# prototypefund/your-voice-TTS

Measured on AMD Instinct MI355X. Metric: mel-frames/sec + RTF, Tacotron2 + 60-iter Griffin-Lim, LJSpeech, higher is better.
Workload: dtype f32; 1 GPU; configs[1]: Tacotron2 single sentence, HIP decoder loop + HIP Griffin-Lim 60 iters; sentences_per_gpu=1, L=100, gl_iters=60, model_config=config_tacotron2.json + forward_attn_mask (synthesize.py:86), parallelism=single GPU

## Files before the change

### your-voice-tts_amd/csrc/resident_decoder.hip

```cpp
#include "handoff.h"
#include "resident.h"

namespace tts {
namespace {
using namespace handoff;

__device__ __forceinline__ float lstm_cell16(float pre, float& c) {
    const int k = threadIdx.x;
    const float act = (k >> 2) == 2 ? tanh_cell(pre) : sigmoid_cell(pre);
    const float f = dpp_move<0x104, 0xf>(act, 0.f);
    const float g = dpp_move<0x108, 0xf>(act, 0.f);
    const float o = dpp_move<0x10C, 0xf>(act, 0.f);
    const float c2 = f * c + act * g;
    c = c2;
    return o * tanh_cell(c2);
}
__device__ __forceinline__ float sigmoid_fast(float x) {
    return __builtin_amdgcn_rcpf(1.f + __builtin_amdgcn_exp2f(-x * 1.4426950408889634f));
}

__device__ __forceinline__ float dot4(float4 w, float4 x, float acc) {
    acc = fmaf(w.x, x.x, acc);
    acc = fmaf(w.y, x.y, acc);
    acc = fmaf(w.z, x.z, acc);
    return fmaf(w.w, x.w, acc);
}
__device__ __forceinline__ float4 ld4(const float* p) { return *reinterpret_cast<const float4*>(p); }
__device__ __forceinline__ float sum32_dpp(float v) {
    v += dpp_move<0x111, 0xf>(v, 0.f);
    v += dpp_move<0x112, 0xf>(v, 0.f);
    v += dpp_move<0x114, 0xf>(v, 0.f);
    v += dpp_move<0x118, 0xf>(v, 0.f);
    v += dpp_move<0x142, 0xa>(v, 0.f);
    return v;
}

__device__ __forceinline__ int res_window(int k, int nn, int L) {
    if (k == 0) return nn >= 2 ? nn - 2 : nn - 2 + L;
    const int clo = nn >= 1 ? nn - 1 : L - 1, chi = min(nn + 2, L - 1);
    const int p = clo + k - 1;
    return p <= chi ? p : -1;
}
__device__ __forceinline__ int res_candidate(int s, int nn, int np, int L) {
    if (s < 5) return res_window(s, nn, L);
    if (s >= 15) return -1;
    const int p = res_window((s - 5) >> 1, np, L);
    if (p < 0) return -1;
    const int q = p + ((s - 5) & 1);
    return q < L ? q : -1;
}

constexpr int SM_WDL = 16 * 16 * 32 * 4;
constexpr int SM_ST = 64;
constexpr int SM_RQ = 4 * 64 * 4;
constexpr int SM_RM = 2 * 6 * 64 * 4 + 2 * 256;
constexpr int SM_PROF = 2 * 16;
constexpr int SM_FLOATS = SM_WDL + HATT + HDEC + (ENC + 16) + PRE + ADIM + 16 + 16 + SM_ST + SM_RQ + SM_RM + SM_PROF + PRE;
static_assert(SM_RM >= 6 * 64 * 4 + RES_WAVES * RES_LMAX, "attention CU partials");
static_assert(SM_RQ >= 3 * RES_LMAX + 2 * RES_WAVES + 16 + ADIM, "attention CU scratch");
static_assert(SM_RQ >= 2 * (RES_LMAX + 32) + RES_LMAX + RES_WAVES, "general attention form: weights, energies");
static_assert(SM_RM >= 2 * 6 * 64 * 4 + RES_LMAX + 32, "general attention form: cumulative weights");
static_assert(RES_LMAX == 4 * 64 && RES_LMAX == 32 * RES_WAVES, "4 positions per lane, one per wave of 32 CUs");

template <bool PROF, bool GEN>
__global__ __launch_bounds__(RES_THREADS, 1) void resident_decoder_kernel(const ResArgs a) {
    const int c = blockIdx.x;
    const int tid = threadIdx.x, lane = tid & 63;
    const int wave = __builtin_amdgcn_readfirstlane(tid >> 6);
    const int r = tid >> 5, ks = tid & 31;
    extern __shared__ __align__(16) float sm[];
    float4* wdl = reinterpret_cast<float4*>(sm);
    float* xh_att = sm + SM_WDL;
    float* xh_dec = xh_att + HATT;
    float* xctx = xh_dec + HDEC;
    float* xpre = xctx + ENC + 16;
    float* xq = xpre + PRE;
    float* gates = xq + ADIM;
    int* flags = reinterpret_cast<int*>(gates + 16);
    float* st = gates + 32;
    float* rq = st + SM_ST;
    float* rm = rq + SM_RQ;
    float* abuf = rq;
    float* an = abuf + 2 * RES_LMAX;
    float* scr = an + RES_LMAX;
    float* xv = scr + 2 * RES_WAVES + 16;
    float* red = rm + 6 * 64 * 4;
    long long* pacc = reinterpret_cast<long long*>(rm + SM_RM);
    float* xp1 = rm + SM_RM + SM_PROF;
    constexpr int GW_PAD = RES_LMAX + 32;
    float* gw = rq;
    float* geg = rq + 2 * GW_PAD;
    float* gts = geg + RES_LMAX;
    float* gcum = rm + 2 * 6 * 64 * 4;
    bool prof = false;
    long long plast = 0;
    long long* trace = PROF && a.prof ? a.prof + 2 * RES_PHASES + (size_t)c * RES_TRACE_STEPS * RES_TRACE_EV : nullptr;
#define RES_EV(t, k)                                                                                \
    if (PROF && trace && (t) < RES_TRACE_STEPS) trace[(t) * RES_TRACE_EV + (k)] = (long long)wall_clock64();
#define RES_MARK(k)                                     \
    if (PROF && prof && tid == 0) {                     \
        const long long now = (long long)wall_clock64(); \
        pacc[k] += now - plast;                         \
        plast = now;                                    \
    }

    float4 wa[14], wdc[4];
    constexpr int KF = HDEC + ENC;
    {
        const float4* p = a.w.wa + (size_t)c * 14 * RES_THREADS + tid;
#pragma unroll
        for (int i = 0; i < 14; ++i) wa[i] = p[(size_t)i * RES_THREADS];
        const float4* q = a.w.wdc + (size_t)c * 4 * RES_THREADS + tid;
#pragma unroll
        for (int i = 0; i < 4; ++i) wdc[i] = q[(size_t)i * RES_THREADS];
        if (wave == 2 && c < a.nmel)
            for (int i = 0; i < 6; ++i) reinterpret_cast<float4*>(rm)[i * 64 + lane] = ld4(a.w.wf + (size_t)c * KF + i * 256 + lane * 4);
        const float4* l = a.w.wdl + (size_t)c * (SM_WDL / 4);
        for (int i = tid; i < SM_WDL / 4; i += RES_THREADS) wdl[i] = l[i];
    }
    if (tid < 16) {
        st[tid] = a.w.ba[c * 16 + tid];
        st[16 + tid] = a.w.bd[c * 16 + tid];
    }
    if (tid < 4) {
        st[32 + tid] = a.c_att[4 * c + tid];
        st[36 + tid] = a.c_dec[4 * c + tid];
    }
    if (tid == 0) st[48] = c < a.nmel ? a.w.bf[c] : 0.f;
    if (tid == 1) st[49] = a.w.bf[a.nmel + PRE];
    for (int k = tid; k < HATT; k += RES_THREADS) {
        xh_att[k] = a.h_att[a.hps + k];
        xh_dec[k] = a.h_dec[a.hps + k];
    }
    for (int k = tid; k < ENC; k += RES_THREADS) xctx[k] = a.xa[PRE + k];
    if (tid == 0) {
        flags[0] = 0;
        flags[1] = 0;
        for (int k = 0; k < RES_PHASES; ++k) pacc[k] = 0;
    }
    __syncthreads();
    const long long tmo = a.timeout_ticks;
    int xcc;
    asm volatile("s_getreg_b32 %0, hwreg(HW_REG_XCC_ID)" : "=s"(xcc));
    xcc &= 7;
    const unsigned setup_tag = (a.salt << 14) | 0x3FFFu;
    if (tid == 0) publish(a.gran + GR_SETUP + c, setup_tag, __int_as_float(xcc));
    if (wave == 0) {
        float v4[4];
        const bool ok = sweep<4>(a.gran, setup_tag, v4, [&](int i) { return GR_SETUP + lane * 4 + i; }, tmo);
        int rank = 0, nx = 0, nmin = RES_CUS, nmax = 0;
        const int xref = __builtin_amdgcn_readfirstlane(__float_as_int(v4[0]) & 7);
        for (int k = 0; k < 8; ++k) {
            int cnt = 0;
#pragma unroll
            for (int i = 0; i < 4; ++i) {
                const int x = __float_as_int(v4[i]) & 7;
                cnt += __popcll(__ballot(x == k));
                if (k == xcc) rank += __popcll(__ballot(x == k && lane * 4 + i < c));
            }
            if (k == xcc) nx = cnt;
            if (cnt > 0) nmin = min(nmin, cnt);
            nmax = max(nmax, cnt);
        }
        if (GEN && nmax > RES_MIN_CUS_PER_XCD) nmin = 0;
        if (lane == 0) {
            int* fl = reinterpret_cast<int*>(flags);
            fl[2] = rank;
            fl[3] = nx;
            fl[4] = xref;
            if (!ok) { flags[1] = 1; fail(a.status, 6); }
            else if (nmin < RES_MIN_CUS_PER_XCD) { flags[1] = 1; fail(a.status, RES_STATUS_PLACEMENT); }
        }
    }
    __syncthreads();
    if (flags[1]) return;
    const int rank = flags[2], nx = flags[3];
    const int p2lo = rank * PRE / nx, p2hi = (rank + 1) * PRE / nx;
    const int r0 = p2lo + wave;
    const bool has_row = r0 < p2hi;
    const float4 wp0 = has_row ? ld4(a.w.w2 + r0 * PRE + lane * 4) : float4{0.f, 0.f, 0.f, 0.f};
    const float bp1 = has_row ? a.w.bf[a.nmel + r0] : 0.f;
    const float bp2 = has_row ? a.w.b2[r0] : 0.f;
    const float* w1p = a.w.wf + (size_t)(a.nmel + (has_row ? r0 : 0)) * KF + lane * 4;
    const bool stop_cu = rank == 0;
    if (stop_cu && wave == 3)
        for (int i = 0; i < 6; ++i)
            reinterpret_cast<float4*>(rm)[(6 + i) * 64 + lane] = ld4(a.w.wf + (size_t)(a.nmel + PRE) * KF + i * 256 + lane * 4);
    const int qrow = 4 * rank + (wave >> 1), qhalf = wave & 1;
    const float4 wq0 = ld4(a.w.wq + qrow * HATT + qhalf * 512 + lane * 4);
    const float4 wq1 = ld4(a.w.wq + qrow * HATT + qhalf * 512 + 256 + lane * 4);
    const int L = a.L;
    const bool att_cu = !GEN && rank == nx - 1;
    const bool xlog = xcc == flags[4];
    const bool att_log = att_cu && xlog;
    prof = PROF && a.prof != nullptr && a.prof_marks && (c == 0 || att_log);
    if (prof && tid == 0) plast = (long long)wall_clock64();
    int n = 0, n_prev = 0;
    float ufa = 0.f, vb = 0.f, ex = 0.f, erow[4] = {0.f, 0.f, 0.f, 0.f}, ptc[4] = {0.f, 0.f, 0.f, 0.f};
    const auto renc = __builtin_amdgcn_make_buffer_rsrc(const_cast<float*>(a.enc), (short)0, L * ENC * 4, 0x00020000);
    const auto rpt = __builtin_amdgcn_make_buffer_rsrc(const_cast<float*>(a.Pt), (short)0, ADIM * a.Lcap * 4, 0x00020000);
    auto prefetch_rows = [&](int nn) {
        const int cx = (nn - 2 + L) % L, clo = nn >= 1 ? nn - 1 : L - 1, chi = min(nn + 2, L - 1);
        ex = __uint_as_float(__builtin_amdgcn_raw_buffer_load_b32(renc, (cx * ENC + tid) * 4, 0, VOLATILE_AUX));
#pragma unroll
        for (int k = 0; k < 4; ++k)
            erow[k] = __uint_as_float(__builtin_amdgcn_raw_buffer_load_b32(
                renc, clo + k <= chi ? ((clo + k) * ENC + tid) * 4 : OOB_OFF, 0, VOLATILE_AUX));
    };
    if (att_cu) {
        n = a.nidx[0];
        ufa = a.u[0];
        vb = a.v_b[0];
        for (int j = tid; j < L; j += RES_THREADS) abuf[j] = a.alpha[j];
        if (tid < ADIM) xv[tid] = a.v[tid];
        prefetch_rows(n);
    }
    const int gf = GEN ? a.gen : 0;
    const int s_e = GR_EX + xcc * RES_LMAX;
    float gu = 0.5f, gtb = 0.f;
    int gwin = -1, gn = 1;
    float gv0 = 0.f, gv1 = 0.f, gp0 = 0.f, gp1 = 0.f, gl0 = 0.f, gl1 = 0.f;
    float gtw[3];
#pragma unroll
    for (int k = 0; k < 3; ++k) gtw[k] = 0.f;
    auto gen_location = [&](const float* wrow) {
        const int pe = rank + 32 * wave;
        if (pe >= L) return;
        const float* src = (lane < 32 ? wrow : gcum) + pe + 1;
        const float4* wc = reinterpret_cast<const float4*>(a.loc_conv) + lane * 8;
        float sacc = 0.f;
#pragma unroll
        for (int q = 0; q < 8; q += 2) {
            const float4 w0 = wc[q], w1_ = wc[q + 1];
            sacc = fmaf(w0.x, src[4 * q], sacc);
            sacc = fmaf(w0.y, src[4 * q + 1], sacc);
            sacc = fmaf(w0.z, src[4 * q + 2], sacc);
            sacc = fmaf(w0.w, src[4 * q + 3], sacc);
            sacc = fmaf(w1_.x, src[4 * q + 4], sacc);
            sacc = fmaf(w1_.y, src[4 * q + 5], sacc);
            sacc = fmaf(w1_.z, src[4 * q + 6], sacc);
            sacc = fmaf(w1_.w, src[4 * q + 7], sacc);
            asm volatile("" ::: "memory");
        }
        const float tot = sacc + __shfl_xor(sacc, 32, 64);
        const float4* wd0 = reinterpret_cast<const float4*>(a.loc_dense + lane * NLOC);
        const float4* wd1 = reinterpret_cast<const float4*>(a.loc_dense + (lane + 64) * NLOC);
        float l0 = 0.f, l1 = 0.f;
#pragma unroll
        for (int q = 0; q < 8; ++q) {
            const float4 u0 = wd0[q], u1 = wd1[q];
            const float f0 = __int_as_float(__builtin_amdgcn_readlane(__float_as_int(tot), 4 * q));
            const float f1 = __int_as_float(__builtin_amdgcn_readlane(__float_as_int(tot), 4 * q + 1));
            const float f2 = __int_as_float(__builtin_amdgcn_readlane(__float_as_int(tot), 4 * q + 2));
            const float f3 = __int_as_float(__builtin_amdgcn_readlane(__float_as_int(tot), 4 * q + 3));
            l0 = fmaf(u0.x, f0, l0); l0 = fmaf(u0.y, f1, l0); l0 = fmaf(u0.z, f2, l0); l0 = fmaf(u0.w, f3, l0);
            l1 = fmaf(u1.x, f0, l1); l1 = fmaf(u1.y, f1, l1); l1 = fmaf(u1.z, f2, l1); l1 = fmaf(u1.w, f3, l1);
            asm volatile("" ::: "memory");
        }
        gl0 = l0;
        gl1 = l1;
    };
    if constexpr (GEN) {
        vb = a.v_b[0];
        gu = a.u[0];
        gn = a.nidx[0];
        if (gf & GEN_WINDOW) gwin = a.win0[0];
        if (gf & GEN_TA) {
            gtb = a.ta_b[0];
#pragma unroll
            for (int k = 0; k < 3; ++k) gtw[k] = a.ta_w[3 * tid + k];
        }
        gv0 = a.v[lane];
        gv1 = a.v[lane + 64];
        const int pe = rank + 32 * wave;
        if (pe < L) {
            gp0 = a.Pt[(int64_t)lane * a.Lcap + pe];
            gp1 = a.Pt[(int64_t)(lane + 64) * a.Lcap + pe];
        }
        for (int k = tid; k < GW_PAD; k += RES_THREADS) {
            const int j = k - 16;
            const bool ok = j >= 0 && j < L;
            gw[k] = ok ? a.alpha[j] : 0.f;
            gw[GW_PAD + k] = ok && (gf & GEN_LOCATION) ? a.att_w0[j] : 0.f;
            gcum[k] = ok && (gf & GEN_LOCATION) ? a.att_cum0[j] : 0.f;
        }
        __syncthreads();
        if (gf & GEN_LOCATION) gen_location(gw + GW_PAD);
    }
    const bool stop_lane = stop_cu && wave == 3 && lane == 0;
    if (stop_lane) {
// ... 22 lines not shown
    int t = 0;
    for (;; ++t) {
        u64* G = a.gran + (t & 1) * GR_TOTAL;
        const unsigned E = (a.salt << 14) | (((unsigned)t & 2047u) << 3);
        const unsigned EP6 = ((a.salt << 14) | (((unsigned)(t - 1) & 2047u) << 3)) + 6u;
        float aa[2] = {0.f, 0.f};
#pragma unroll
        for (int i = 2; i < 6; ++i) aa[i & 1] = dot4(wa[i], ld4(xctx + (i - 2) * 128 + ks * 4), aa[i & 1]);
#pragma unroll
        for (int i = 6; i < 10; ++i) aa[i & 1] = dot4(wa[i], ld4(xh_att + (i - 6) * 128 + ks * 4), aa[i & 1]);
        asm volatile("" ::: "memory");
#pragma unroll
        for (int i = 10; i < 14; ++i) aa[i & 1] = dot4(wa[i], ld4(xh_att + (i - 6) * 128 + ks * 4), aa[i & 1]);
        float acc_a = aa[0] + aa[1];
        float ad[2] = {0.f, 0.f};
#pragma unroll 2
        for (int i = 8; i < 16; ++i)
            ad[i & 1] = dot4(wdl[(i * 16 + r) * 32 + ks], ld4(xh_dec + (i - 8) * 128 + ks * 4), ad[i & 1]);
        float acc_d = ad[0] + ad[1];
        if (wave < 3) {
            const int gp = s_1 + ((t & 1) ^ 1) * GR_TOTAL;
            bool ok = true;
            if (t == 0) {
                if (wave == 0) {
                    const float4 v = ld4(a.pre1 + lane * 4);
                    xp1[lane * 4] = v.x; xp1[lane * 4 + 1] = v.y; xp1[lane * 4 + 2] = v.z; xp1[lane * 4 + 3] = v.w;
                }
            } else {
                float p0 = 0.f, p1 = 0.f;
                for (int i = 0; i < a.sleep_p1; ++i) __builtin_amdgcn_s_sleep(4);
                if (wave < 2) {
                    ok = sweep_pair(rg, gp + 2 * pk, true, EP6, p0, p1, tmo);
                    xp1[2 * pk] = p0;
                    xp1[2 * pk + 1] = p1;
                } else {
                    ok = sweep_pair(rg, lane == 0 ? gp + PRE : -1, false, EP6, p0, p1, tmo);
                    if (lane == 0 && ok && p0 == 0.f) flags[0] = 1;
                }
            }
            RES_MARK(0);
            if (lane == 0 && !ok) { flags[1] = 1; fail(a.status, 1, t); }
        }
        __syncthreads();
        if (tid == 0) { RES_EV(t, 0) }
        if (flags[0] | flags[1]) break;
        {
            const float4 x = ld4(xp1 + lane * 4);
            u64* gx = Gx + (t & 1) * GR_TOTAL;
            if (has_row) {
                const float s0 = wave_sum_dpp(dot4(wp0, x, 0.f));
                if (lane == 0) publish_xcd(gx + r0, E + 1, fmaxf(s0 + bp2, 0.f));
            }
            RES_MARK(1);
            if (wave < 2) {
                for (int i = 0; i < a.sleep_pre2; ++i) __builtin_amdgcn_s_sleep(4);
                float q0, q1;
                const bool ok = sweep_pair(rg, s_x + (t & 1) * GR_TOTAL + 2 * pk, true, E + 1, q0, q1, tmo);
                xpre[2 * pk] = q0;
                xpre[2 * pk + 1] = q1;
                if (!ok && lane == 0) { flags[1] = 1; fail(a.status, 7, t); }
            }
        }
        __syncthreads();
        if (tid == 0) { RES_EV(t, 1) }
        if (flags[1]) break;
        RES_MARK(2);
#pragma unroll
        for (int i = 0; i < 2; ++i) acc_a = dot4(wa[i], ld4(xpre + i * 128 + ks * 4), acc_a);
        acc_a = sum32_dpp(acc_a);
        if (ks == 31) gates[r] = acc_a;
        __syncthreads();
        RES_MARK(3);
        if (tid < 16) {
            float cs = st[32 + (tid & 3)];
            const float h = lstm_cell16(gates[tid] + st[tid], cs);
            if (tid < 4) {
                st[32 + tid] = cs;
                st[40 + tid] = h;
                publish(G + GR_HATT + 4 * c + tid, E + 2, h);
                if (tid == 0) { RES_EV(t, 2) }
            }
        }
        if (att_cu && t > 0) {
            prefetch_rows(n);
            const int pos = res_candidate(tid >> 5, n, n_prev, L);
#pragma unroll
            for (int m = 0; m < 4; ++m)
                ptc[m] = __uint_as_float(__builtin_amdgcn_raw_buffer_load_b32(
                    rpt, pos >= 0 ? (((tid & 31) + 32 * m) * a.Lcap + pos) * 4 : OOB_OFF, 0, VOLATILE_AUX));
        }
        {
            if (wave == 4 && t > 0) mel_row(t - 1);
            for (int i = 0; i < a.sleep_hatt; ++i) __builtin_amdgcn_s_sleep(4);
            float h0, h1;
            const bool ok = sweep_pair(rg, (t & 1) * GR_TOTAL + GR_HATT + 2 * pk, true, E + 2, h0, h1, tmo);
            xh_att[2 * pk] = h0;
            xh_att[2 * pk + 1] = h1;
            if (!ok && lane == 0) { flags[1] = 1; fail(a.status, 2, t); }
        }
        __syncthreads();
        if (tid == 0) { RES_EV(t, 3) }
        if (flags[1]) break;
        RES_MARK(4);
        {
            float s = dot4(wq0, ld4(xh_att + qhalf * 512 + lane * 4), 0.f);
            s = dot4(wq1, ld4(xh_att + qhalf * 512 + 256 + lane * 4), s);
            s = wave_sum_dpp(s);
            if (lane == 0) publish_xcd(Gq + (t & 1) * GR_TOTAL + 2 * qrow + qhalf, E + 3, s);
            if (tid == 0) { RES_EV(t, 8) }
        }
        if (!att_cu) {
#pragma unroll 2
            for (int i = 0; i < 8; ++i) acc_d = dot4(wdl[(i * 16 + r) * 32 + ks], ld4(xh_att + i * 128 + ks * 4), acc_d);
        }
        RES_MARK(5);
        float wdef = 0.f;
        if constexpr (GEN) {
            float2 gen_e[4];
#pragma unroll
            for (int i = 0; i < 4; ++i) {
                const int ps = (i >> 1) * 128 + 2 * lane + (i & 1);
                gen_e[i] = __builtin_bit_cast(float2, __builtin_amdgcn_raw_buffer_load_b64(
                    renc, ps < L ? (ps * ENC + 16 * rank + 2 * wave) * 4 : OOB_OFF, 0, VOLATILE_AUX));
            }
            if (wave < 2) {
                for (int i = 0; i < a.sleep_q; ++i) __builtin_amdgcn_s_sleep(1);
                float q0, q1;
                const bool ok = sweep_pair(rg, s_q + (t & 1) * GR_TOTAL + 2 * pk, true, E + 3, q0, q1, tmo);
                xq[pk] = q0 + q1;
                if (!ok && lane == 0) { flags[1] = 1; fail(a.status, 3, t); }
            }
            __syncthreads();
            if (flags[1]) break;
            if (rank + 32 * wave < L) {
                float x0 = xq[lane], x1 = xq[lane + 64];
                if (gf & GEN_LOCATION) {
                    x0 += gl0;
                    x1 += gl1;
                }
                const float e = wave_sum_dpp(gv0 * tanh_fast(x0 + gp0) + gv1 * tanh_fast(x1 + gp1));
                if (lane == 0) publish_xcd(a.gran + (t & 1) * GR_TOTAL + s_e + rank + 32 * wave, E + 7, e + vb);
            }
            if (wave < 2) {
                for (int i = 0; i < a.sleep_e; ++i) __builtin_amdgcn_s_sleep(1);
                const int p0 = 2 * pk;
                float e0 = 0.f, e1 = 0.f;
                const bool ok =
                    sweep_pair(rg, p0 < L ? s_e + (t & 1) * GR_TOTAL + p0 : -1, p0 + 1 < L, E + 7, e0, e1, tmo);
                geg[p0] = e0;
                geg[p0 + 1] = e1;
                if (!ok && lane == 0) { flags[1] = 1; fail(a.status, 8, t); }
            }
            __syncthreads();
            if (flags[1]) break;
            RES_MARK(6);
            const float* wold = gw + (t & 1) * GW_PAD + 16;
            float* wnew = gw + ((t & 1) ^ 1) * GW_PAD + 16;
            int ps[4];
            bool in[4];
            float e[4];
            {
                const float2 g0 = *reinterpret_cast<const float2*>(geg + 2 * lane);
                const float2 g1 = *reinterpret_cast<const float2*>(geg + 128 + 2 * lane);
                e[0] = g0.x; e[1] = g0.y; e[2] = g1.x; e[3] = g1.y;
            }
#pragma unroll
            for (int i = 0; i < 4; ++i) {
                ps[i] = (i >> 1) * 128 + 2 * lane + (i & 1);
                in[i] = ps[i] < L;
                if (!in[i]) e[i] = -INFINITY;
            }
            if (gf & GEN_WINDOW) {
                const int back = gwin - 2, front = gwin + 6;
#pragma unroll
                for (int i = 0; i < 4; ++i)
                    if (in[i] && ((back > 0 && ps[i] < back) || (front < L && ps[i] >= front))) e[i] = -INFINITY;
                if (gwin == -1) {
                    const float m = wave_max_dpp(fmaxf(fmaxf(e[0], e[1]), fmaxf(e[2], e[3])));
                    if (lane == 0) e[0] = m;
                }
                float bv = e[0];
                int bi = ps[0];
#pragma unroll
                for (int i = 1; i < 4; ++i)
                    if (e[i] > bv) { bv = e[i]; bi = ps[i]; }
                wave_argmax(bv, bi);
                gwin = __builtin_amdgcn_readfirstlane(bi);
            }
            float al[4];
            if (gf & GEN_SOFTMAX) {
                const float m = wave_max_dpp(fmaxf(fmaxf(e[0], e[1]), fmaxf(e[2], e[3])));
#pragma unroll
                for (int i = 0; i < 4; ++i) al[i] = in[i] ? expf(e[i] - m) : 0.f;
            } else {
#pragma unroll
                for (int i = 0; i < 4; ++i) al[i] = in[i] ? sigmoidf_(e[i]) : 0.f;
            }
            {
                const float S = wave_sum_dpp((al[0] + al[1]) + (al[2] + al[3]));
#pragma unroll
                for (int i = 0; i < 4; ++i) al[i] = al[i] / S;
            }
            if ((gf & GEN_LOCATION) && wave == 0) {
                float2* c01 = reinterpret_cast<float2*>(gcum + 16 + 2 * lane);
                float2* c23 = reinterpret_cast<float2*>(gcum + 16 + 128 + 2 * lane);
                const float2 o01 = *c01, o23 = *c23;
                *c01 = float2{o01.x + al[0], o01.y + al[1]};
                *c23 = float2{o23.x + al[2], o23.y + al[3]};
            }
            float w[4];
            if (gf & GEN_FORWARD) {
                float an[4];
#pragma unroll
                for (int i = 0; i < 4; ++i) {
                    const float ao = wold[ps[i]], pv = wold[ps[i] - 1];
                    const float mix = __fadd_rn(__fadd_rn(__fmul_rn(1.f - gu, ao), __fmul_rn(gu, pv)), 1e-8f);
                    an[i] = in[i] ? __fmul_rn(mix, al[i]) : 0.f;
                }
                if (gf & GEN_MASK) {
                    const float rmax = wave_max_dpp(fmaxf(fmaxf(in[0] ? an[0] : -INFINITY, in[1] ? an[1] : -INFINITY),
                                                          fmaxf(in[2] ? an[2] : -INFINITY, in[3] ? an[3] : -INFINITY)));
                    const int cx = gn >= 2 ? gn - 2 : gn - 2 + L, lo = gn >= 1 ? gn - 1 : L - 1;
#pragma unroll
                    for (int i = 0; i < 4; ++i) {
                        const bool keep = in[i] && ps[i] < gn + 3 && ps[i] >= lo;
                        an[i] = ps[i] == cx ? 0.01f * rmax : (keep ? an[i] : 0.f);
                    }
                }
                const float denom = wave_sum_dpp((an[0] + an[1]) + (an[2] + an[3]));
#pragma unroll
                for (int i = 0; i < 4; ++i) w[i] = in[i] ? an[i] / denom : 0.f;
                if (gf & GEN_MASK) {
                    float bv = -1.f;
                    int bi = 0x7fffffff;
#pragma unroll
                    for (int i = 0; i < 4; ++i)
                        if (ps[i] <= L - 2 && w[i] > bv) { bv = w[i]; bi = ps[i]; }
                    wave_argmax(bv, bi);
                    gn = __builtin_amdgcn_readfirstlane(bv > 0.f ? bi + 1 : 0);
                }
            } else {
#pragma unroll
                for (int i = 0; i < 4; ++i) w[i] = al[i];
            }
            RES_MARK(7);
            const float tail = wave_sum_dpp(((ps[0] >= L - 2 && in[0] ? w[0] : 0.f) + (ps[1] >= L - 2 && in[1] ? w[1] : 0.f)) +
                                            ((ps[2] >= L - 2 && in[2] ? w[2] : 0.f) + (ps[3] >= L - 2 && in[3] ? w[3] : 0.f)));
            float c0 = 0.f, c1 = 0.f;
#pragma unroll
            for (int i = 0; i < 4; ++i) {
                c0 = fmaf(w[i], gen_e[i].x, c0);
                c1 = fmaf(w[i], gen_e[i].y, c1);
            }
            c0 = wave_sum_dpp(c0);
            c1 = wave_sum_dpp(c1);
            {
                u64* gcx = Gc + (t & 1) * GR_TOTAL;
                if (lane < 2) publish_xcd(gcx + 16 * rank + 2 * wave + lane, E + 4, lane ? c1 : c0);
                if (rank == 0 && wave == 0 && lane == 2) publish_xcd(gcx + ENC, E + 4, tail);
            }
            if (tid == 0) { RES_EV(t, 11) }
            RES_MARK(8);
            if (wave == 0) {
                *reinterpret_cast<float2*>(wnew + 2 * lane) = float2{w[0], w[1]};
                *reinterpret_cast<float2*>(wnew + 128 + 2 * lane) = float2{w[2], w[3]};
                if (xlog && rank == 0 && t < a.hist_cap) {
#pragma unroll
                    for (int i = 0; i < 4; ++i)
                        if (ps[i] < a.Lalign) a.align_hist[(int64_t)t * a.Lalign + ps[i]] = w[i];
                }
            }
        }
        if (att_cu) {
            const float* aold = abuf + (t & 1) * RES_LMAX;
            float* anew = abuf + ((t & 1) ^ 1) * RES_LMAX;
            float* candv = scr + 2 * RES_WAVES;
            const int cx = n >= 2 ? n - 2 : n - 2 + L, clo = n >= 1 ? n - 1 : L - 1, chi = min(n + 2, L - 1);
            const int sl = tid >> 5, sub = tid & 31;
            const int pos = t > 0 ? res_candidate(sl, n, n_prev, L) : -1;
            float xvd[4];
#pragma unroll
            for (int m = 0; m < 4; ++m) xvd[m] = xv[sub + 32 * m];
            const float a_pos = pos >= 0 ? aold[pos] : 0.f, a_prev = pos > 0 ? aold[pos - 1] : 0.f;
            if (wave < 2) {
                for (int i = 0; i < a.sleep_q; ++i) __builtin_amdgcn_s_sleep(1);
                float q0, q1;
                const bool ok = sweep_pair(rg, s_q + (t & 1) * GR_TOTAL + 2 * pk, true, E + 3, q0, q1, tmo);
                xq[pk] = q0 + q1;
                if (!ok && lane == 0) { flags[1] = 1; fail(a.status, 3, t); }
            }
            __syncthreads();
            if (tid == 0) { RES_EV(t, 9) }
            if (flags[1]) break;
            RES_MARK(6);
            bool full = t == 0;
            float rm = -INFINITY, cand = -INFINITY;
            if (!full) {
                float part = 0.f;
#pragma unroll
                for (int m = 0; m < 4; ++m) part += xvd[m] * tanh_fast(xq[sub + 32 * m] + ptc[m]);
                const float e = sum32_dpp(part);
                if (sub == 31) {
                    float v = -INFINITY;
                    if (pos >= 0) {
                        const float sg = sigmoid_fast(e + vb);
                        const float mix = __fadd_rn(__fadd_rn(__fmul_rn(1.f - ufa, a_pos), __fmul_rn(ufa, a_prev)), 1e-8f);
                        v = __fmul_rn(mix, sg);
                        an[pos] = v;
                    }
                    candv[sl] = v;
                }
                __syncthreads();
                if (tid == 0) { RES_EV(t, 10) }
                RES_MARK(14);
                cand = candv[lane & 15];
                rm = wave_max_dpp(cand);
                full = !(rm >= 1e-8f);
            }
            if (full) {
                float xqd[16];
#pragma unroll
                for (int dd = 0; dd < 16; ++dd) xqd[dd] = xq[16 * wave + dd];
#pragma unroll 1
                for (int jj = lane; jj < L; jj += 64) {
                    float s = 0.f;
#pragma unroll
                    for (int dd = 0; dd < 16; ++dd) {
                        const int d = 16 * wave + dd;
                        s += xv[d] * tanh_fast(xqd[dd] + a.Pt[(int64_t)d * a.Lcap + jj]);
                    }
                    red[wave * RES_LMAX + jj] = s;
                }
                __syncthreads();
                const int j = tid;
                float anj = -INFINITY;
                if (j < L) {
                    float e = 0.f;
#pragma unroll
                    for (int w = 0; w < RES_WAVES; ++w) e += red[w * RES_LMAX + j];
                    const float sg = sigmoid_fast(e + vb);
                    const float prev = j > 0 ? aold[j - 1] : 0.f;
                    const float mix = __fadd_rn(__fadd_rn(__fmul_rn(1.f - ufa, aold[j]), __fmul_rn(ufa, prev)), 1e-8f);
                    anj = __fmul_rn(mix, sg);
                    an[j] = anj;
                }
                const float wmax = wave_max_dpp(anj);
                if (lane == 0) scr[2 * wave + 1] = wmax;
                __syncthreads();
                rm = -INFINITY;
#pragma unroll
                for (int k = 0; k < RES_WAVES; ++k) rm = fmaxf(rm, scr[2 * k + 1]);
            }
            RES_MARK(7);
            float aw[4];
#pragma unroll
            for (int k = 0; k < 4; ++k) {
                const float c = full ? an[clo + k] : __int_as_float(__builtin_amdgcn_readlane(__float_as_int(cand), 1 + k));
                aw[k] = (clo + k <= chi && clo + k != cx) ? c : 0.f;
            }
            const float rs = ((aw[0] + aw[1]) + aw[2]) + aw[3];
            const float vx = 0.01f * rm;
            const float denom = rs + vx;
            const float inv = 1.f / denom;
            const float wcx = vx * inv;
            float ww[4];
#pragma unroll
            for (int k = 0; k < 4; ++k) ww[k] = aw[k] * inv;
            auto weight = [&](int p) -> float {
                if (p == cx) return wcx;
                return (p >= clo && p <= chi) ? ww[p - clo] : 0.f;
            };
            const float tail = weight(L - 2) + weight(L - 1);
            float bv = 0.f;
            int bi = -1;
            auto consider = [&](int p) {
                const float wp = weight(p);
                if (p <= L - 2 && wp > bv) { bv = wp; bi = p; }
            };
            if (cx < clo) consider(cx);
#pragma unroll
            for (int k = 0; k < 4; ++k)
                if (clo + k <= chi) consider(clo + k);
            if (cx > chi) consider(cx);
            float ctx = 0.f;
            if (cx < clo) ctx += wcx * ex;
#pragma unroll
            for (int k = 0; k < 4; ++k)
                if (clo + k <= chi) ctx += (clo + k == cx ? wcx * ex : ww[k] * erow[k]);
            if (cx > chi) ctx += wcx * ex;
            RES_MARK(15);
            publish_xcd(Gc + (t & 1) * GR_TOTAL + tid, E + 4, ctx);
            if (tid == 0) publish_xcd(Gc + (t & 1) * GR_TOTAL + ENC, E + 4, tail);
            xctx[tid] = ctx;
            if (tid == 0) xctx[ENC] = tail;
            if (tid == 0) { RES_EV(t, 11) }
            RES_MARK(8);
            wdef = tid < L ? weight(tid) : 0.f;
            n_prev = n;
            n = bi >= 0 ? bi + 1 : 0;
#pragma unroll
            for (int h = 0; h < 2; ++h) {
                float4 wv[4], xv4[4];
#pragma unroll
                for (int j = 0; j < 4; ++j) {
                    wv[j] = wdl[((4 * h + j) * 16 + r) * 32 + ks];
                    xv4[j] = ld4(xh_att + (4 * h + j) * 128 + ks * 4);
                }
#pragma unroll
                for (int j = 0; j < 4; ++j) acc_d = dot4(wv[j], xv4[j], acc_d);
                asm volatile("" ::: "memory");
            }
            RES_MARK(9);
        }
        float4 w1[6];
#pragma unroll
        for (int i = 0; i < 6; ++i) w1[i] = ld4(w1p + i * 256);
        if (wave < 5 && !att_cu) {
            const int gc = s_c + (t & 1) * GR_TOTAL;
            for (int i = 0; i < a.sleep_ctx; ++i) __builtin_amdgcn_s_sleep(4);
            float c0 = 0.f, c1 = 0.f;
            const bool ok = wave < 4 ? sweep_pair(rg, gc + 2 * pk, true, E + 4, c0, c1, tmo)
                                     : sweep_pair(rg, lane == 0 ? gc + ENC : -1, false, E + 4, c0, c1, tmo);
            if (wave < 4) {
                xctx[2 * pk] = c0;
                xctx[2 * pk + 1] = c1;
            } else if (lane == 0) {
                xctx[ENC] = c0;
            }
            if (!ok && lane == 0) { flags[1] = 1; fail(a.status, 4, t); }
        }
        __syncthreads();
        if (tid == 0) { RES_EV(t, 4) }
        if (flags[1]) break;
        RES_MARK(10);
#pragma unroll
        for (int i = 0; i < 4; ++i) acc_d = dot4(wdc[i], ld4(xctx + i * 128 + ks * 4), acc_d);
        acc_d = sum32_dpp(acc_d);
        if (ks == 31) gates[r] = acc_d;
        __syncthreads();
        RES_MARK(11);
        if (tid < 16) {
            float cs = st[36 + (tid & 3)];
            const float h = lstm_cell16(gates[tid] + st[16 + tid], cs);
            if (tid < 4) {
                st[36 + tid] = cs;
                st[44 + tid] = h;
                publish(G + GR_HDEC + 4 * c + tid, E + 5, h);
                if (tid == 0) { RES_EV(t, 5) }
            }
        }
        if constexpr (GEN) {
            if (gf & GEN_TA) {
                float pta = 0.f;
#pragma unroll
                for (int k = 0; k < 3; ++k) {
                    const int idx = 3 * tid + k;
                    pta = fmaf(gtw[k], idx < ENC ? xctx[idx] : xh_att[idx - ENC], pta);
                }
                pta = wave_sum_dpp(pta);
                if (lane == 0) gts[wave] = pta;
            }
            if (gf & GEN_LOCATION) gen_location(gw + ((t & 1) ^ 1) * GW_PAD);
        }
        if (att_cu) {
            float* anew = abuf + ((t & 1) ^ 1) * RES_LMAX;
            if (tid < L) anew[tid] = wdef;
            if (att_log && t < a.hist_cap && tid < a.Lalign) a.align_hist[(int64_t)t * a.Lalign + tid] = wdef;
        }
        {
            for (int i = 0; i < a.sleep_hdec; ++i) __builtin_amdgcn_s_sleep(4);
            float h0, h1;
            const bool ok = sweep_pair(rg, (t & 1) * GR_TOTAL + GR_HDEC + 2 * pk, true, E + 5, h0, h1, tmo);
            xh_dec[2 * pk] = h0;
            xh_dec[2 * pk + 1] = h1;
            if (!ok && lane == 0) { flags[1] = 1; fail(a.status, 5, t); }
        }
        __syncthreads();
        if (tid == 0) { RES_EV(t, 6) }
        if (flags[1]) break;
        if constexpr (GEN) {
            if (gf & GEN_TA) {
                float sta = gts[0];
#pragma unroll
                for (int k = 1; k < RES_WAVES; ++k) sta += gts[k];
                gu = sigmoidf_(sta + gtb);
            }
        }
        RES_MARK(12);
        long long m0 = 0;
        if (prof && tid == 128) m0 = (long long)wall_clock64();
        {
            const bool stw = stop_cu && wave == 3;
            const float4* wsr = reinterpret_cast<const float4*>(rm) + 6 * 64 + lane;
            float s = 0.f, ss = 0.f;
#pragma unroll
            for (int i = 0; i < 4; ++i) {
                const float4 x = ld4(xh_dec + i * 256 + lane * 4);
                s = dot4(w1[i], x, s);
                if (stw) ss = dot4(wsr[i * 64], x, ss);
            }
#pragma unroll
            for (int i = 4; i < 6; ++i) {
                const float4 x = ld4(xctx + (i - 4) * 256 + lane * 4);
                s = dot4(w1[i], x, s);
                if (stw) ss = dot4(wsr[i * 64], x, ss);
            }
            s = wave_sum_dpp(s);
            u64* g1 = G1 + (t & 1) * GR_TOTAL;
            if (has_row && lane == 0) {
                const float p = fmaxf(s + bp1, 0.f);
                publish_xcd(g1 + r0, E + 6, p);
                if (wave == 0) { RES_EV(t, 7) }
                if (xlog) a.pre1[r0] = p;
            }
            if (stw) {
                ss = wave_sum_dpp(ss);
                if (lane == 0) {
                    const float stv = sigmoidf_(ss + st[49]);
                    if (xlog && t < a.hist_cap) a.stop_hist[t] = stv;
                    const float tail = xctx[ENC];
                    int* sst = reinterpret_cast<int*>(st);
                    const int f1 = sst[50] | ((tail > 0.8f && t > L) ? 1 : 0);
                    sst[50] = f1;
                    int nd = 0;
                    if (f1 && t > 2 * L) {
                        sst[51] += 1;
                        if (sst[51] > 20) nd = 1;
                    } else if (t + 1 == a.max_steps) {
                        nd = 1;
                    }
                    if (!nd && t + 1 >= a.hist_cap) {
                        nd = 1;
                        fail(a.status, 100);
                    }
                    if (nd && xlog) {
                        a.done[0] = 1;
                        a.n_steps[0] = t + 1;
                    }
                    publish_xcd(g1 + PRE, E + 6, nd ? 0.f : 1.f);
                }
            }
        }
        if (prof && tid == 128) pacc[13] += (long long)wall_clock64() - m0;
    }
    if (flags[1]) return;
    if (wave == 4 && t > 0) mel_row(t - 1);
    if (prof && tid == 0)
        for (int k = 0; k < RES_PHASES; ++k) a.prof[(c == 0 ? 0 : 1) * RES_PHASES + k] = pacc[k];
// ... 125 lines not shown
```

### your-voice-tts_amd/tacotron2.py

```python
from __future__ import annotations

import ctypes
from collections import OrderedDict

import numpy as np
import torch

from . import _native, weights


def _speaker_array(speaker_ids, B):
    spk = np.asarray(torch.as_tensor(speaker_ids).view(-1).cpu().numpy(), dtype=np.int32)
    if spk.size == 1 and B > 1:
        spk = np.repeat(spk, B)
    if spk.size != B:
        raise ValueError(f"speaker_ids has {spk.size} entries for a batch of {B}")
    return np.ascontiguousarray(spk)


class _DecoderAttrs:

    def __init__(self, r):
        self.max_decoder_steps = 1000
        self.r = r
# ... 258 lines not shown
    def inference(self, text, speaker_ids=None):
        text = torch.as_tensor(text)
        if text.dim() == 1:
            text = text.unsqueeze(0)
        out = self.inference_batch([row for row in text.cpu().numpy()], speaker_ids=speaker_ids)
        return out["mel"], out["mel_post"], out["align"], out["stop"].unsqueeze(-1)

    @torch.no_grad()
    def synthesize_native(self, ids_list, ap, seed=0, iters=None, sync=True, speaker_ids=None, out=None):
        if speaker_ids is not None and "speaker_embedding.weight" not in self._params:
            speaker_ids = None
        lens = [len(x) for x in ids_list]
        if min(lens) < 2:
            raise ValueError("encoder length must be >= 2 (common_layers.py:213)")
        B, Lmax = len(lens), max(lens)
        lib, hdec, hpost = self._handles(Lmax, B)
        _, hgl = ap._handle()
        key = (self._native[2], id(ap), hgl.value if hasattr(hgl, "value") else int(hgl))
        if self._synth is not None and self._synth[1] != key:
            lib.tts_synth_destroy(self._synth[0])
            self._synth = None
        if self._synth is None:
            hs = ctypes.c_void_p()
            _native.check(lib.tts_synth_create(self._native[3], hdec, hpost, hgl, self.n_frames_per_step, 80,
                                               ap.hop_length, ctypes.byref(hs)), "tts_synth_create")
            self._synth = (hs, key, ap)
        hs = self._synth[0]
        max_steps = int(self.decoder.max_decoder_steps)
        ids = np.zeros((B, Lmax), np.int32)
        for b, x in enumerate(ids_list):
            ids[b, :lens[b]] = np.asarray(x, dtype=np.int32)
        cap = self.native_wav_capacity(ap, B)
        if out is not None:
            if out.dtype != torch.float64 or not out.is_cuda or not out.is_contiguous() or out.numel() < cap:
                raise ValueError(f"out must be a contiguous CUDA float64 buffer of >= {cap} elements")
            wav_buf = out
        else:
            if self._wav_buf is None or self._wav_buf.numel() < cap:
                self._wav_buf = torch.empty(cap, dtype=torch.float64, device=self.device)
            wav_buf = self._wav_buf
        frames = (ctypes.c_int32 * B)()
        iters = ap.griffin_lim_iters if iters is None else iters
        if speaker_ids is None:
            _native.check(lib.tts_synth_run(hs, ids.ctypes.data_as(_native.I32P), _native.i32_array(lens), B, Lmax,
                                            max_steps, int(iters), int(seed), ctypes.c_void_p(wav_buf.data_ptr()),
                                            cap, frames, _native.stream_handle()), "tts_synth_run")
        else:
            spk = _speaker_array(speaker_ids, B)
            _native.check(lib.tts_synth_run_speakers(hs, ids.ctypes.data_as(_native.I32P), _native.i32_array(lens),
                                                     _native.i32_array(spk), B, Lmax, max_steps, int(iters), int(seed),
                                                     ctypes.c_void_p(wav_buf.data_ptr()), cap, frames,
                                                     _native.stream_handle()), "tts_synth_run_speakers")
        frames = [int(f) for f in frames]
        if sync:
            _native.check(lib.tts_synth_sync(hs), "tts_synth_sync")
        self.last_timing = self._path_timing(lib, hdec)
        self.last_lengths = frames
        n = ap.hop_length * (max(frames) - 1)
        return wav_buf.view(-1)[:B * n].view(B, n), frames

    def native_wav_capacity(self, ap, B=1):
        return B * ap.hop_length * ((int(self.decoder.max_decoder_steps) + 21) * self.n_frames_per_step - 1)

    def resident_limits(self, Lmax=1):
        lib, hdec, _ = self._handles(max(int(Lmax), 1), 1)
        mb, ml = ctypes.c_int(), ctypes.c_int()
        _native.check(lib.tts_decoder_resident_limits(hdec, ctypes.byref(mb), ctypes.byref(ml)),
                      "tts_decoder_resident_limits")
        return mb.value, ml.value

    def synth_sync(self):
        if self._synth is not None:
            _native.check(_native.lib().tts_synth_sync(self._synth[0]), "tts_synth_sync")

    def _path_timing(self, lib, hdec):
        ms, ns, res, enc = ctypes.c_float(), ctypes.c_int(), ctypes.c_int(), ctypes.c_int()
        lib.tts_decoder_last_timing(hdec, ctypes.byref(ms), ctypes.byref(ns))
        lib.tts_decoder_last_path(hdec, ctypes.byref(res))
        lib.tts_encoder_last_path(self._native[3], ctypes.byref(enc))
        return dict(decoder_loop_ms=ms.value, decoder_steps_run=ns.value, resident=bool(res.value),
                    resident_kind=int(res.value), encoder_resident=bool(enc.value), encoder_path=int(enc.value))

    RESIDENT_PHASES = ("att_early_wait_pre1", "prenet2_row", "wait_prenet2", "att_lstm_prenet", "att_cell_gather",
                       "query_dec_early", "wait_query", "energies_max", "weights_ctx_publish", "next_prefetch",
                       "wait_ctx", "dec_lstm_ctx", "dec_cell_gather", "fused_rows", "cand_energies", "weights_ctx")

    def profile_resident_phases(self):
        lib, hdec, _ = self._handles(1, 1)
        n = 2 * len(self.RESIDENT_PHASES)
        us = (ctypes.c_float * n)()
        _native.check(lib.tts_decoder_resident_phases(hdec, us, n), "tts_decoder_resident_phases")
        k = len(self.RESIDENT_PHASES)
        return {"cu0": dict(zip(self.RESIDENT_PHASES, [float(v) for v in us[:k]])),
                "attention_cu": dict(zip(self.RESIDENT_PHASES, [float(v) for v in us[k:]]))}

    def profile_resident_trace(self):
        lib, hdec, _ = self._handles(1, 1)
        n = 256 * 64 * 12
        buf = (ctypes.c_longlong * n)()
        _native.check(lib.tts_decoder_resident_trace(hdec, buf, n), "tts_decoder_resident_trace")
        return np.frombuffer(buf, dtype=np.int64).reshape(256, 64, 12).copy()

    def profile_step_kernels(self, reps=50):
        lib, hdec, _ = self._handles(1, 1)
        n = len(_native.DECODER_STEP_KERNELS)
        ms = (ctypes.c_float * n)()
        _native.check(lib.tts_decoder_profile(hdec, int(reps), ms, n), "tts_decoder_profile")
        return dict(zip(_native.DECODER_STEP_KERNELS, [float(v) for v in ms]))

    @torch.no_grad()
    def inference_truncated(self, text, speaker_ids=None):
        _native.lib()
        text = torch.as_tensor(text)
        if text.dim() == 1:
            text = text.unsqueeze(0)
        if text.shape[0] != 1:
            raise ValueError("inference_truncated is batch-1 (the reference keeps one state per module)")
        L = int(text.shape[1])
        lib, _, _ = self._handles(L, 1)
        if self.flags["forward_attn_mask"] and L < 2:
            raise ValueError("encoder length must be >= 2 with forward_attn_mask")
        ids32 = text.to(self.device, dtype=torch.int32).contiguous()
        enc = torch.empty(1, L, 512, device=self.device)
        state_out = torch.empty(4, 1, 256, device=self.device)
        st_in = self._enc_state
        _native.check(lib.tts_encoder_run_state(
            self._native[3], ctypes.c_void_p(ids32.data_ptr()), _native.i32_array([L]), 1, L,
            ctypes.c_void_p(st_in.data_ptr()) if st_in is not None else None, ctypes.c_void_p(state_out.data_ptr()),
            ctypes.c_void_p(enc.data_ptr()), _native.stream_handle()), "tts_encoder_run_state")
        self._enc_state = state_out
        if speaker_ids is not None and "speaker_embedding.weight" in self._params:
            self._add_speakers(lib, enc, [L], speaker_ids)
        out = self.inference_batch(None, enc=enc, lens=[L], _continue=self._trunc_started)
        self._trunc_started = True
        return out["mel"], out["mel_post"], out["align"], out["stop"].unsqueeze(-1)

    __call__ = inference
```

Before: 96370 mel-frames/s.

## Shorten attention-CU critical path: reuse encoder rows, hoist mix, defer weight writes

On the attention CU, the encoder rows for the next window are now shifted in registers when the attention index advances by one, so only one new row is loaded instead of five. The decoder-LSTM hatt dot product moves ahead of the attention wait rather than running after context publication. The forward-attention mix term is computed before the query wait, and the per-position weight writeback moves out of the context-publish section. The goal is to shorten the serial attention step that gates every decoder step, at the cost of more live registers and more restructured control logic.

```diff
diff --git a/your-voice-tts_amd/csrc/resident_decoder.hip b/your-voice-tts_amd/csrc/resident_decoder.hip
--- a/your-voice-tts_amd/csrc/resident_decoder.hip
+++ b/your-voice-tts_amd/csrc/resident_decoder.hip
@@ -48,6 +48,72 @@
     if (p < 0) return -1;
     const int q = p + ((s - 5) & 1);
     return q < L ? q : -1;
+}
+
+struct ResWin {
+    int cx, clo, chi;
+    bool in[4];
+    bool iscx[4];
+    bool pre, post;
+};
+__device__ __forceinline__ ResWin res_win(int n, int L) {
+    ResWin w;
+    w.cx = n >= 2 ? n - 2 : n - 2 + L;
+    w.clo = n >= 1 ? n - 1 : L - 1;
+    w.chi = min(n + 2, L - 1);
+#pragma unroll
+    for (int k = 0; k < 4; ++k) {
+        w.in[k] = w.clo + k <= w.chi;
+        w.iscx[k] = w.in[k] && w.clo + k == w.cx;
+    }
+    w.pre = w.cx < w.clo;
+    w.post = w.cx > w.chi;
+    return w;
+}
+__device__ __forceinline__ void res_weights(const ResWin& w, float rm, const float (&c)[4], float& wcx, float (&ww)[4]) {
+    float aw[4];
+#pragma unroll
+    for (int k = 0; k < 4; ++k) aw[k] = (w.in[k] && !w.iscx[k]) ? c[k] : 0.f;
+    const float rs = ((aw[0] + aw[1]) + aw[2]) + aw[3];
+    const float vx = 0.01f * rm;
+    const float denom = rs + vx;
+    const float inv = 1.f / denom;
+    wcx = vx * inv;
+#pragma unroll
+    for (int k = 0; k < 4; ++k) ww[k] = aw[k] * inv;
+}
+__device__ __forceinline__ float res_context(const ResWin& w, float wcx, const float (&ww)[4], float ex,
+                                             const float (&erow)[4]) {
+    const float px = wcx * ex;
+    float ctx = 0.f;
+    ctx = w.pre ? ctx + px : ctx;
+#pragma unroll
+    for (int k = 0; k < 4; ++k) {
+        const float s = ctx + (w.iscx[k] ? px : ww[k] * erow[k]);
+        ctx = w.in[k] ? s : ctx;
+    }
+    ctx = w.post ? ctx + px : ctx;
+    return ctx;
+}
+__device__ __forceinline__ float res_weight_at(const ResWin& w, float wcx, const float (&ww)[4], int p) {
+    const int d = p - w.clo;
+    const float v = d == 0 ? ww[0] : d == 1 ? ww[1] : d == 2 ? ww[2] : ww[3];
+    return p == w.cx ? wcx : ((p >= w.clo && p <= w.chi) ? v : 0.f);
+}
+__device__ __forceinline__ int res_tail_next(const ResWin& w, float wcx, const float (&ww)[4], int L, float& tail) {
+    tail = res_weight_at(w, wcx, ww, L - 2) + res_weight_at(w, wcx, ww, L - 1);
+    float bv = 0.f;
+    int bi = -1;
+    auto consider = [&](bool present, int p, float wp) {
+        const bool take = present && p <= L - 2 && wp > bv;
+        bv = take ? wp : bv;
+        bi = take ? p : bi;
+    };
+    consider(w.pre, w.cx, wcx);
+#pragma unroll
+    for (int k = 0; k < 4; ++k) consider(w.in[k], w.clo + k, w.iscx[k] ? wcx : ww[k]);
+    consider(w.post, w.cx, wcx);
+    return bi >= 0 ? bi + 1 : 0;
 }
 
 constexpr int SM_WDL = 16 * 16 * 32 * 4;
@@ -200,12 +266,25 @@
     const auto renc = __builtin_amdgcn_make_buffer_rsrc(const_cast<float*>(a.enc), (short)0, L * ENC * 4, 0x00020000);
     const auto rpt = __builtin_amdgcn_make_buffer_rsrc(const_cast<float*>(a.Pt), (short)0, ADIM * a.Lcap * 4, 0x00020000);
     auto prefetch_rows = [&](int nn) {
-        const int cx = (nn - 2 + L) % L, clo = nn >= 1 ? nn - 1 : L - 1, chi = min(nn + 2, L - 1);
+        const int cx = nn >= 2 ? nn - 2 : nn - 2 + L, clo = nn >= 1 ? nn - 1 : L - 1, chi = min(nn + 2, L - 1);
         ex = __uint_as_float(__builtin_amdgcn_raw_buffer_load_b32(renc, (cx * ENC + tid) * 4, 0, VOLATILE_AUX));
 #pragma unroll
         for (int k = 0; k < 4; ++k)
             erow[k] = __uint_as_float(__builtin_amdgcn_raw_buffer_load_b32(
                 renc, clo + k <= chi ? ((clo + k) * ENC + tid) * 4 : OOB_OFF, 0, VOLATILE_AUX));
+    };
+    auto advance_rows = [&](int from, int nn) {
+        if (nn == from) return;
+        if (nn == from + 1 && from >= 1) {
+            ex = erow[0];
+            erow[0] = erow[1];
+            erow[1] = erow[2];
+            erow[2] = erow[3];
+            erow[3] = __uint_as_float(__builtin_amdgcn_raw_buffer_load_b32(
+                renc, nn + 2 <= L - 1 ? ((nn + 2) * ENC + tid) * 4 : OOB_OFF, 0, VOLATILE_AUX));
+        } else {
+            prefetch_rows(nn);
+        }
     };
     if (att_cu) {
         n = a.nidx[0];
@@ -394,7 +473,7 @@
             }
         }
         if (att_cu && t > 0) {
-            prefetch_rows(n);
+            advance_rows(n_prev, n);
             const int pos = res_candidate(tid >> 5, n, n_prev, L);
 #pragma unroll
             for (int m = 0; m < 4; ++m)
@@ -421,12 +500,11 @@
             if (lane == 0) publish_xcd(Gq + (t & 1) * GR_TOTAL + 2 * qrow + qhalf, E + 3, s);
             if (tid == 0) { RES_EV(t, 8) }
         }
-        if (!att_cu) {
 #pragma unroll 2
-            for (int i = 0; i < 8; ++i) acc_d = dot4(wdl[(i * 16 + r) * 32 + ks], ld4(xh_att + i * 128 + ks * 4), acc_d);
-        }
+        for (int i = 0; i < 8; ++i) acc_d = dot4(wdl[(i * 16 + r) * 32 + ks], ld4(xh_att + i * 128 + ks * 4), acc_d);
         RES_MARK(5);
-        float wdef = 0.f;
+        float wcx = 0.f, ww[4] = {0.f, 0.f, 0.f, 0.f};
+        int n_win = 0;
         if constexpr (GEN) {
             float2 gen_e[4];
 #pragma unroll
@@ -585,15 +663,16 @@
         }
         if (att_cu) {
             const float* aold = abuf + (t & 1) * RES_LMAX;
-            float* anew = abuf + ((t & 1) ^ 1) * RES_LMAX;
             float* candv = scr + 2 * RES_WAVES;
-            const int cx = n >= 2 ? n - 2 : n - 2 + L, clo = n >= 1 ? n - 1 : L - 1, chi = min(n + 2, L - 1);
+            const ResWin win = res_win(n, L);
             const int sl = tid >> 5, sub = tid & 31;
             const int pos = t > 0 ? res_candidate(sl, n, n_prev, L) : -1;
             float xvd[4];
 #pragma unroll
             for (int m = 0; m < 4; ++m) xvd[m] = xv[sub + 32 * m];
             const float a_pos = pos >= 0 ? aold[pos] : 0.f, a_prev = pos > 0 ? aold[pos - 1] : 0.f;
+            const float mix = __fadd_rn(__fadd_rn(__fmul_rn(1.f - ufa, a_pos), __fmul_rn(ufa, a_prev)), 1e-8f);
+            RES_MARK(9);
             if (wave < 2) {
                 for (int i = 0; i < a.sleep_q; ++i) __builtin_amdgcn_s_sleep(1);
                 float q0, q1;
@@ -606,28 +685,26 @@
             if (flags[1]) break;
             RES_MARK(6);
             bool full = t == 0;
-            float rm = -INFINITY, cand = -INFINITY;
+            float rm = -INFINITY;
+            float cw[4] = {0.f, 0.f, 0.f, 0.f};
             if (!full) {
                 float part = 0.f;
 #pragma unroll
                 for (int m = 0; m < 4; ++m) part += xvd[m] * tanh_fast(xq[sub + 32 * m] + ptc[m]);
                 const float e = sum32_dpp(part);
                 if (sub == 31) {
-                    float v = -INFINITY;
-                    if (pos >= 0) {
-                        const float sg = sigmoid_fast(e + vb);
-                        const float mix = __fadd_rn(__fadd_rn(__fmul_rn(1.f - ufa, a_pos), __fmul_rn(ufa, a_prev)), 1e-8f);
-                        v = __fmul_rn(mix, sg);
-                        an[pos] = v;
-                    }
+                    const float v = pos >= 0 ? __fmul_rn(mix, sigmoid_fast(e + vb)) : -INFINITY;
+                    if (pos >= 0) an[pos] = v;
                     candv[sl] = v;
                 }
                 __syncthreads();
                 if (tid == 0) { RES_EV(t, 10) }
                 RES_MARK(14);
-                cand = candv[lane & 15];
+                const float cand = candv[lane & 15];
                 rm = wave_max_dpp(cand);
                 full = !(rm >= 1e-8f);
+#pragma unroll
+                for (int k = 0; k < 4; ++k) cw[k] = __int_as_float(__builtin_amdgcn_readlane(__float_as_int(cand), 1 + k));
             }
             if (full) {
                 float xqd[16];
@@ -652,8 +729,8 @@
                     for (int w = 0; w < RES_WAVES; ++w) e += red[w * RES_LMAX + j];
                     const float sg = sigmoid_fast(e + vb);
                     const float prev = j > 0 ? aold[j - 1] : 0.f;
-                    const float mix = __fadd_rn(__fadd_rn(__fmul_rn(1.f - ufa, aold[j]), __fmul_rn(ufa, prev)), 1e-8f);
-                    anj = __fmul_rn(mix, sg);
+                    const float mixj = __fadd_rn(__fadd_rn(__fmul_rn(1.f - ufa, aold[j]), __fmul_rn(ufa, prev)), 1e-8f);
+                    anj = __fmul_rn(mixj, sg);
                     an[j] = anj;
                 }
                 const float wmax = wave_max_dpp(anj);
@@ -662,67 +739,24 @@
                 rm = -INFINITY;
 #pragma unroll
                 for (int k = 0; k < RES_WAVES; ++k) rm = fmaxf(rm, scr[2 * k + 1]);
+#pragma unroll
+                for (int k = 0; k < 4; ++k) cw[k] = an[win.clo + k];
             }
             RES_MARK(7);
-            float aw[4];
-#pragma unroll
-            for (int k = 0; k < 4; ++k) {
-                const float c = full ? an[clo + k] : __int_as_float(__builtin_amdgcn_readlane(__float_as_int(cand), 1 + k));
-                aw[k] = (clo + k <= chi && clo + k != cx) ? c : 0.f;
-            }
-            const float rs = ((aw[0] + aw[1]) + aw[2]) + aw[3];
-            const float vx = 0.01f * rm;
-            const float denom = rs + vx;
-            const float inv = 1.f / denom;
-            const float wcx = vx * inv;
-            float ww[4];
-#pragma unroll
-            for (int k = 0; k < 4; ++k) ww[k] = aw[k] * inv;
-            auto weight = [&](int p) -> float {
-                if (p == cx) return wcx;
-                return (p >= clo && p <= chi) ? ww[p - clo] : 0.f;
-            };
-            const float tail = weight(L - 2) + weight(L - 1);
-            float bv = 0.f;
-            int bi = -1;
-            auto consider = [&](int p) {
-                const float wp = weight(p);
-                if (p <= L - 2 && wp > bv) { bv = wp; bi = p; }
-            };
-            if (cx < clo) consider(cx);
-#pragma unroll
-            for (int k = 0; k < 4; ++k)
-                if (clo + k <= chi) consider(clo + k);
-            if (cx > chi) consider(cx);
-            float ctx = 0.f;
-            if (cx < clo) ctx += wcx * ex;
-#pragma unroll
-            for (int k = 0; k < 4; ++k)
-                if (clo + k <= chi) ctx += (clo + k == cx ? wcx * ex : ww[k] * erow[k]);
-            if (cx > chi) ctx += wcx * ex;
+            res_weights(win, rm, cw, wcx, ww);
+            const float ctx = res_context(win, wcx, ww, ex, erow);
             RES_MARK(15);
             publish_xcd(Gc + (t & 1) * GR_TOTAL + tid, E + 4, ctx);
+            xctx[tid] = ctx;
+            if (tid == 0) { RES_EV(t, 11) }
+            float tail;
+            const int n_next = res_tail_next(win, wcx, ww, L, tail);
             if (tid == 0) publish_xcd(Gc + (t & 1) * GR_TOTAL + ENC, E + 4, tail);
-            xctx[tid] = ctx;
             if (tid == 0) xctx[ENC] = tail;
-            if (tid == 0) { RES_EV(t, 11) }
             RES_MARK(8);
-            wdef = tid < L ? weight(tid) : 0.f;
+            n_win = n;
             n_prev = n;
-            n = bi >= 0 ? bi + 1 : 0;
-#pragma unroll
-            for (int h = 0; h < 2; ++h) {
-                float4 wv[4], xv4[4];
-#pragma unroll
-                for (int j = 0; j < 4; ++j) {
-                    wv[j] = wdl[((4 * h + j) * 16 + r) * 32 + ks];
-                    xv4[j] = ld4(xh_att + (4 * h + j) * 128 + ks * 4);
-                }
-#pragma unroll
-                for (int j = 0; j < 4; ++j) acc_d = dot4(wv[j], xv4[j], acc_d);
-                asm volatile("" ::: "memory");
-            }
-            RES_MARK(9);
+            n = n_next;
         }
         float4 w1[6];
 #pragma unroll
@@ -776,6 +810,7 @@
         }
         if (att_cu) {
             float* anew = abuf + ((t & 1) ^ 1) * RES_LMAX;
+            const float wdef = tid < L ? res_weight_at(res_win(n_win, L), wcx, ww, tid) : 0.f;
             if (tid < L) anew[tid] = wdef;
             if (att_log && t < a.hist_cap && tid < a.Lalign) a.align_hist[(int64_t)t * a.Lalign + tid] = wdef;
         }
diff --git a/your-voice-tts_amd/tacotron2.py b/your-voice-tts_amd/tacotron2.py
--- a/your-voice-tts_amd/tacotron2.py
+++ b/your-voice-tts_amd/tacotron2.py
@@ -364,7 +364,7 @@
                     resident_kind=int(res.value), encoder_resident=bool(enc.value), encoder_path=int(enc.value))
 
     RESIDENT_PHASES = ("att_early_wait_pre1", "prenet2_row", "wait_prenet2", "att_lstm_prenet", "att_cell_gather",
-                       "query_dec_early", "wait_query", "energies_max", "weights_ctx_publish", "next_prefetch",
+                       "query_dec_early", "wait_query", "energies_max", "weights_ctx_publish", "dec_lstm_hatt",
                        "wait_ctx", "dec_lstm_ctx", "dec_cell_gather", "fused_rows", "cand_energies", "weights_ctx")
 
     def profile_resident_phases(self):
```

Result: faster. 97440 mel-frames/s (median of 6 runs) (+1.1%).
